# jwscook/DistributedHouseholderQR.jl

Measured on AMD Instinct MI355X. Metric: QR GFLOP/s (F = 2mn^2 - 2/3 n^3), ||A-QR||/||A|| alongside, higher is better.
Workload: dtype f64; 1 GPU; 32768x32768 Float64 dense QR, blocked nb=128 (BASELINE configs[2]); m=32768, n=32768, nb=128, parallelism=single GPU

## Files before the change

### distributedhouseholderqr.jl_amd/_lib.py

```python
from __future__ import annotations

import ctypes
import os
import subprocess

_PKG = os.path.dirname(os.path.abspath(__file__))
SO_PATH = os.path.join(_PKG, "libdhqr.so")
BENCH_SO_PATH = os.path.join(_PKG, "libdhqr_bench.so")
CSRC = os.path.join(_PKG, "csrc")
NB = 128
CS_BLOCK = 256
ZNB = 64

OK, EINVAL, EHIP, ENOMEM, ENODEVICE, ECOMM = 0, -1, -2, -3, -4, -5
COMM_SELF, COMM_RCCL, COMM_LOCAL, COMM_CALLBACK = 0, 1, 2, 3
UNIQUE_ID_BYTES = 128


class DHQRError(RuntimeError):
    def __init__(self, code: int, msg: str):
        super().__init__(f"libdhqr error {code}: {msg}")
        self.code = code


# ... 96 lines not shown
    "dhqr_cs_store_contiguous_f64": (_i32, [_p, _p, _i64, _i64, _i64, _p, _i64, _p]),
    "dhqr_cs_qr_darray_f64": (_i32, [_p, _p, _i64, _i64, _i64, _p]),
    "dhqr_mg_create": (_i32, [_pp, _pi32, _i32]),
    "dhqr_mg_destroy": (_i32, [_p]),
    "dhqr_mg_info": (_i32, [_p, _pi32, _pi32, _pi64, _pi64]),
    "dhqr_mg_get_bcast_tuning": (_i32, [_p, _pi32, _pd, _pd]),
    "dhqr_mg_rccl_nranks": (_i32, [_p, _pi32, _pi32]),
    "dhqr_mg_comm_counters": (_i32, [_p, _i32, _pi64]),
    "dhqr_mg_alloc_f64": (_i32, [_p, _i64, _i64]),
    "dhqr_mg_fill_uniform_f64": (_i32, [_p, _u64]),
    "dhqr_mg_factor_f64": (_i32, [_p]),
    "dhqr_mg_residual_f64": (_i32, [_p, _u64, _pd]),
    "dhqr_mg_upload_f64": (_i32, [_p, _p, _i64, _p]),
    "dhqr_mg_download_f64": (_i32, [_p, _p, _i64, _p]),
    "dhqr_mg_qr_f64": (_i32, [_p, _p, _i64, _i64, _i64, _p]),
    "dhqr_mg_qr_c64": (_i32, [_p, _p, _i64, _i64, _i64, _p]),
    "dhqr_cs_local_cols_c64": (_i64, [_i64, _i32, _i32]),
    "dhqr_cs_factor_c64": (_i32, [_p, _p, _i64, _i64, _i64, _p]),
    "dhqr_cs_qr_darray_c64": (_i32, [_p, _p, _i64, _i64, _i64, _p]),
    "dhqr_comm_timing": (_i32, [_p, _i32, _p]),
    "dhqr_mg_comm_timing": (_i32, [_p, _i32, _i32, _p]),
    "dhqr_cs_ldiv_darray_f64": (_i32, [_p, _p, _i64, _i64, _i64, _p, _p, _p]),
    "dhqr_cs_ldiv_darray_c64": (_i32, [_p, _p, _i64, _i64, _i64, _p, _p, _p]),
    "dhqr_cs_solve_work_c64": (_i64, [_i64, _i32]),
    "dhqr_cs_solve_c64": (_i32, [_p, _p, _i64, _i64, _i64, _p, _p, _p]),
    "dhqr_mg_ldiv_c64": (_i32, [_p, _p, _i64, _i64, _i64, _p, _p, _p]),
    "dhqr_mg_solve_f64": (_i32, [_p, _p, _p]),
    "dhqr_mg_ldiv_f64": (_i32, [_p, _p, _i64, _i64, _i64, _p, _p, _p]),
    "dhqr_mg_set_profiling": (_i32, [_p, _i32]),
    "dhqr_mg_reset_stats": (_i32, [_p]),
    "dhqr_mg_get_stats": (_i32, [_p, _i32, ctypes.POINTER(Stats), _pi64, _pi64, _pi64]),
    "dhqr_rs_row_range": (None, [_i64, _i32, _i32, _pi64, _pi64]),
    "dhqr_rs_fill_uniform_f64": (_i32, [_p, _p, _i64, _i64, _i64, _u64]),
    "dhqr_rs_factor_f64": (_i32, [_p, _p, _i64, _i64, _i64, _p]),
    "dhqr_rs_residual_f64": (_i32, [_p, _p, _i64, _i64, _i64, _p, _u64, _p, _p, _pd]),
    "dhqr_rs_solve_f64": (_i32, [_p, _p, _i64, _i64, _i64, _p, _p, _p]),
    "dhqr_mg_rs_alloc_f64": (_i32, [_p, _i64, _i64]),
    "dhqr_mg_rs_fill_uniform_f64": (_i32, [_p, _u64]),
    "dhqr_mg_rs_factor_f64": (_i32, [_p]),
    "dhqr_mg_rs_residual_f64": (_i32, [_p, _u64, _pd]),
    "dhqr_mg_rs_transfer_f64": (_i32, [_p, _p, _i64, _p, _i32]),
    "dhqr_mg_rs_solve_f64": (_i32, [_p, _p, _p]),
}

BENCH_SIGNATURES = {
    "dhqr_bench_mfma_f64": (_i32, [_p, _pd]),
    "dhqr_bench_issue_f64": (_i32, [_p, _i32, _i32, _pd, _pd]),
    "dhqr_bench_issue2_f64": (_i32, [_p, _i32, _i32, _i32, _pd]),
    "dhqr_bench_stream_f64": (_i32, [_p, _i64, _pd]),
    "dhqr_debug_mfma_probe": (_i32, [_p, _p, _p, _p]),
    "dhqr_bench_gemm_f64": (_i32, [_p, _i32, _i64, _i64, _i32, _pd]),
    "dhqr_bench_mma_probe_f64": (_i32, [_p, _i32, _i32, _pd]),
    "dhqr_bench_lane_probe_f64": (_i32, [_p, _i64, _i32, _i32, _i32, _pd]),
    "dhqr_debug_hold_cus": (_i32, [_p, _i32, _i32, _i32]),
    "dhqr_debug_smq_phases": (_i32, [_p, _pd]),
}

_lib = None


def lib() -> ctypes.CDLL:
    global _lib
    if _lib is None:
        if not os.path.exists(SO_PATH):
            raise ImportError(
                f"{SO_PATH} not found: build it with __graft_entry__.build() "
                "(hipcc --offload-arch=gfx950); this package has no CPU fallback")
        L = ctypes.CDLL(SO_PATH)
        for name, (res, args) in SIGNATURES.items():
            fn = getattr(L, name)
            fn.restype = res
            fn.argtypes = args
        _lib = L
    return _lib


_bench = None


def lib_bench() -> ctypes.CDLL:
    global _bench
    if _bench is None:
        if not os.path.exists(BENCH_SO_PATH):
            raise ImportError(f"{BENCH_SO_PATH} not found: build it with __graft_entry__.build()")
        L = ctypes.CDLL(BENCH_SO_PATH)
        for name, (res, args) in list(SIGNATURES.items()) + list(BENCH_SIGNATURES.items()):
            fn = getattr(L, name)
            fn.restype = res
            fn.argtypes = args
        _bench = L
    return _bench


def check(rc: int) -> None:
    if rc != OK:
        raise DHQRError(rc, lib().dhqr_last_error().decode(errors="replace"))
```

### distributedhouseholderqr.jl_amd/csrc/dhqr_api.hip

```cpp
#include <chrono>
#include <mutex>

#include "dhqr_internal.h"
#include "dhqr_complex.h"
#include "dhqr_gemm.h"
#include "dhqr_pack.h"
#include "dhqr_panel.h"
#include "dhqr_recon.h"
#include "dhqr_solve.h"
#include "dhqr_qtb.h"
#include "dhqr_small.h"
#include "dhqr_batched.h"
#include "dhqr_tsqr.h"

static thread_local char g_err[512] = "";
int32_t set_err(int32_t code, const char *fmt, ...) {
  va_list ap;
  va_start(ap, fmt);
  vsnprintf(g_err, sizeof(g_err), fmt, ap);
  va_end(ap);
  return code;
}
int32_t ensure(dhqr_ctx *c, Buf &b, size_t need) {
  if (need <= b.cap) return DHQR_OK;
  if (b.p) {
    HIPCHECK(hipDeviceSynchronize());
    HIPCHECK(hipFree(b.p));
    b.p = nullptr;
    b.cap = 0;
  }
  need = (need + 1023) & ~(size_t)1023;
  hipError_t e = hipMalloc((void **)&b.p, need * sizeof(double));
  if (e != hipSuccess)
    return set_err(DHQR_ENOMEM, "hipMalloc(%zu bytes) failed: %s", need * sizeof(double),
                   hipGetErrorString(e));
  b.cap = need;
  return DHQR_OK;
}

bool tune_get(const char *key, long long *out) {
  const char *e = getenv("DHQR_TUNE");
  if (!e) return false;
  const size_t kl = strlen(key);
  for (const char *p = e; *p;) {
    const char *q = strchr(p, ',');
    const size_t len = q ? (size_t)(q - p) : strlen(p);
    if (len > kl + 1 && strncmp(p, key, kl) == 0 && p[kl] == '=') {
      *out = atoll(p + kl + 1);
      return true;
    }
    if (!q) break;
    p = q + 1;
  }
  return false;
}

static std::atomic<int> g_live_ctx[64];


int32_t prof_begin(dhqr_ctx *c, int cat) {
  if (!c->profiling) return DHQR_OK;
// ... 527 lines not shown
                                    const PanelBuf &pb, int panel_idx, int part = 0) {
  const size_t NN = (size_t)DHQR_NBV * DHQR_NBV;
  const double *Rref = panel_rbuf(c, panel_idx) + 3 * NN, *altmp = panel_rbuf(c, panel_idx) + 6 * NN;
  if (part == 1) {
    hipLaunchKernelGGL(k_commit_alpha, dim3(1), dim3(DHQR_NBV), 0, stream, altmp, (int)DHQR_NBV, (double *)nullptr, pb.alpha,
                       (const int *)c->dstat, panel_idx);
  } else {
    dim3 grid((unsigned)std::min<int64_t>((rows + 255) / 256, 64), DHQR_NBV);
    hipLaunchKernelGGL(k_commit_panel, grid, dim3(256), 0, stream, P, ldp, rows, (const double *)pb.V, pb.ldv, Rref, altmp, alpha,
                       part == 2 ? (double *)nullptr : pb.alpha, (const int *)c->dstat, panel_idx);
  }
  LAUNCHCHECK();
  return DHQR_OK;
}
static int32_t panel_fast_enqueue(dhqr_ctx *c, double *P, int64_t rows, int64_t ldp, double *alpha, const PanelBuf &pb,
                                  int passes, int panel_idx, hipEvent_t ev_v = nullptr, hipEvent_t ev_t = nullptr) {
  const int64_t ldv = pb.ldv;
  const size_t NN = (size_t)DHQR_NBV * DHQR_NBV;
  CHECK(ensure(c, c->rbuf, 2 * panel_rbuf_elems()));
  if (passes == 2) CHECK(ensure(c, c->vts, (size_t)panel_elems(rows)));
  if (passes == 3) CHECK(ensure(c, c->tsq, TsqrLocal::elems(rows)));
  CHECK(ensure(c, c->sfull, NN));
  if (c->ev_commit[panel_idx & 1]) HIPCHECK(hipStreamWaitEvent(c->stream, c->ev_commit[panel_idx & 1], 0));
  double *R1 = panel_rbuf(c, panel_idx), *negR1inv = R1 + NN, *Rf = R1 + 2 * NN, *Rref = R1 + 3 * NN, *negMinv = R1 + 4 * NN;
  double *G = R1 + 5 * NN, *altmp = R1 + 6 * NN;
  int *bflag = c->dstat + 1;
  CHECK(prof_begin(c, CAT_PANEL));
  const bool was = c->profiling;
  c->profiling = false;
  auto body = [&]() -> int32_t {
    const double *X = P;
    int64_t ldx = ldp;
    if (passes == 3) {
      TsqrLocal t;
      t.place(c->tsq.p, rows);
      CHECK(tsqr_local_up(c, t, P, ldp, Rf, true));
      CHECK(tsqr_local_down(c, t, nullptr));
      hipLaunchKernelGGL(k_tsqr_identity, dim3((unsigned)(NN / 256)), dim3(256), 0, c->stream, R1);
      X = t.Yl;
      ldx = t.ldy;
      launch_recon_top(c, X, ldx, R1, G, Rref, negMinv);
      hipLaunchKernelGGL(k_tsqr_sign_cols, dim3((unsigned)(NN / 256)), dim3(256), 0, c->stream, negMinv, (const double *)Rf);
    } else if (passes == 2) {
      CHECK(gram128(c, P, ldp, rows, G));
      double *Q1 = c->vts.p;
      const int64_t ldq = panel_ldv(rows);
      launch_chol_inv(c, G, nullptr, R1, negR1inv, bflag);
      CHECK(mul128(c, P, ldp, rows, negR1inv, Q1, ldq));
      CHECK(gram128(c, Q1, ldq, rows, G));
      launch_chol_inv(c, G, R1, Rf, nullptr, bflag);
      launch_recon_top(c, P, ldp, Rf, altmp, Rref, negMinv);
    } else {
      CHECK(gram128(c, P, ldp, rows, G));
      hipLaunchKernelGGL((k_panel_top<false>), dim3(1), dim3(1024), 0, c->stream, (const double *)G, (const double *)P, ldp, altmp,
                         Rref, negMinv, bflag);
    }
    if (c->fuse_fix) {
      CHECK(mul128(c, X, ldx, rows, negMinv, pb.V, ldv, passes == 3 ? G : altmp));
    } else {
      CHECK(mul128(c, X, ldx, rows, negMinv, pb.V, ldv));
      hipLaunchKernelGGL(k_recon_fix, dim3(NN / 256), dim3(256), 0, c->stream, pb.V, ldv,
                         (const double *)(passes == 3 ? G : altmp), (const double *)negMinv);
    }
    if (ev_v) HIPCHECK(hipEventRecord(ev_v, c->stream));
    if (passes == 3)
      hipLaunchKernelGGL(k_tsqr_final_r, dim3(NN / 256), dim3(256), 0, c->stream, (const double *)Rf, (const double *)G, Rref,
                         altmp);
    CHECK(gram128(c, pb.V, ldv, rows, c->sfull.p));
    hipLaunchKernelGGL(k_build_t, dim3(1), dim3(1024), 0, c->stream, (const double *)c->sfull.p, (int)DHQR_NBV, pb.T, pb.Tt,
                       c->recon_tol, c->dstat, panel_idx, pb.alpha + DHQR_NBV, c->tt_keep);
    if (ev_t) HIPCHECK(hipEventRecord(ev_t, c->stream));
    else CHECK(panel_commit_enqueue(c, c->stream, P, rows, ldp, alpha, pb, panel_idx));
    LAUNCHCHECK();
    return DHQR_OK;
  };
  const int32_t rc = body();
  c->profiling = was;
  CHECK(rc);
  if (c->profiling)
    for (int64_t j = 0; j + 1 < DHQR_NBV; ++j) c->st.bytes_panel += 16.0 * (double)(rows - j) * (double)(DHQR_NBV - j - 1);
  CHECK(prof_end(c));
  return DHQR_OK;
}
static inline bool panel_fast_eligible(dhqr_ctx *c, int64_t rows, int64_t w) {
  return c->panel_impl == 3 && w == DHQR_NBV && rows >= 2 * DHQR_NBV;
}

static int32_t factor_panel_sync(dhqr_ctx *c, double *P, int64_t rows, int64_t w, int64_t ldp, double *alpha,
                                 const PanelBuf &pb) {
  if (panel_fast_eligible(c, rows, w)) {
    const int last_rung = std::max(c->cholqr_passes, c->tsqr_rung == 1 ? 3 : 2);
    for (int passes = c->cholqr_passes; passes <= last_rung; ++passes) {
      CHECK(status_reset(c));
      CHECK(panel_fast_enqueue(c, P, rows, ldp, alpha, pb, passes, 0));
      int failed = 0;
      CHECK(status_read(c, &failed));
      if (failed == INT_MAX) {
        c->n_fast++;
        if (passes == 3) c->n_tsqr++;
        return DHQR_OK;
      }
    }
    CHECK(status_reset(c));
    c->n_fallback++;
  }
  if (c->panel_impl >= 2 && !(c->partial_unblocked && rows > 256 && rows <= c->partial_unblocked_max_rows))
    return factor_panel_v2(c, P, rows, w, ldp, alpha, pb);
  CHECK(factor_unblocked_cols(c, P, rows, w, ldp, alpha, CAT_PANEL));
  return panel_pack_and_t(c, P, rows, w, ldp, alpha, pb);
}

static int32_t comm_allreduce_sum(dhqr_comm *cm, double *dbuf, int64_t count, hipStream_t stream);

static inline int64_t nn_row_chunks(const dhqr_ctx *c, int64_t row_tiles) {
  if (c->nn_split <= 1 || c->cur_ws != 0) return 1;
  return std::max<int64_t>(1, std::min<int64_t>(c->nn_split, row_tiles / c->nn_chunk_tiles));
}

static int32_t narrow_vtc(dhqr_ctx *c, const double *Vp, int64_t ldv, int64_t rows, const double *C, int64_t ldc,
                          int64_t ncols, bool vec, Buf &part, double *Y) {
  const int64_t ntiles = (ncols + 127) / 128, ld2 = 2 * DHQR_NBV, wstride = ld2 * ncols;
  int64_t nsplit, rps;
  pick_split(rows, 2 * ntiles, 512, 256 / ntiles, &nsplit, &rps, 512, 64);
// ... 419 lines not shown
  HIPCHECK(hipGetDeviceProperties(&prop, device));
  if (strncmp(prop.gcnArchName, "gfx950", 6) != 0)
    return set_err(DHQR_ENODEVICE, "device %d is %s; this library is built for gfx950 only", device,
                   prop.gcnArchName);
  dhqr_ctx *c = new dhqr_ctx();
  c->device = device;
  c->coop = prop.cooperativeLaunch != 0;
  g_live_ctx[device & 63].fetch_add(1);
  memset(&c->st, 0, sizeof(c->st));
  auto init = [&]() -> int32_t {
    HIPCHECK(hipStreamCreateWithFlags(&c->own, hipStreamNonBlocking));
    c->stream = c->own;
    {
      int lo = 0, hi = 0;
      HIPCHECK(hipDeviceGetStreamPriorityRange(&lo, &hi));
      HIPCHECK(hipStreamCreateWithPriority(&c->hi, hipStreamNonBlocking, hi));
      if (const char *e = getenv("DHQR_LANE_SIDE")) c->lane_side = atoi(e) != 0;
      c->hi_priority = hi;
    }
    if (const char *e = getenv("DHQR_LOOKAHEAD")) c->lookahead = atoi(e) != 0;
    {
      int ncu = 0;
      if (hipDeviceGetAttribute(&ncu, hipDeviceAttributeMultiprocessorCount, device) == hipSuccess && ncu > 0) {
        c->rankk_wgs = ncu;
        c->ncu = ncu;
      }
    }
    if (const char *e = getenv("DHQR_SPARE_CUS")) {
      c->spare_cus = std::max(0, std::min(c->ncu - 8, atoi(e)));
      c->spare_cus_set = true;
    }
    if (const char *e = getenv("DHQR_QUAD")) c->quad = atoi(e) != 0;
    if (const char *e = getenv("DHQR_QUAD_MIN_COLS")) c->quad_min_cols = std::max<int64_t>(0, atoll(e));
    { long long v; if (tune_get("rankk_wgs", &v)) c->rankk_wgs = std::max(2, (int)v); }
    if (const char *e = getenv("DHQR_RANKK")) c->rankk = c->rankk_tall = c->rankk_xtall = std::min(5, std::max(1, atoi(e)));
    if (const char *e = getenv("DHQR_RANKK_MAX")) c->rankk_max = std::min(DHQR_RK_KMAX, std::max(1, atoi(e)));
    { long long v; if (tune_get("rankk_max_min_cols", &v)) c->rankk_max_min_cols = std::max(0, (int)v); }
    { long long v; if (tune_get("nn_chunk_tiles", &v)) c->nn_chunk_tiles = std::max(1, (int)v); }
    if (const char *e = getenv("DHQR_NN_SPLIT")) c->nn_split = std::min(16, std::max(1, atoi(e)));
    if (const char *e = getenv("DHQR_RANKK_PIPE")) c->rankk_pipe = std::min(2, std::max(0, atoi(e)));
    { long long v; if (tune_get("tn_min_tiles", &v)) c->tn_model_min_tiles = (int)v; }
    { long long v; if (tune_get("small_flags", &v)) c->small_flags = v != 0; }
    { long long v; if (tune_get("batched_wave", &v)) c->batched_wave = v != 0; }
    { long long v; if (tune_get("short_panel_small", &v)) c->short_panel_small = v != 0; }
    { long long v; if (tune_get("partial_unblocked", &v)) c->partial_unblocked = v != 0; }
    { long long v; if (tune_get("partial_unblocked_max_rows", &v)) c->partial_unblocked_max_rows = v; }
    { long long v; if (tune_get("small_spin_limit", &v)) c->small_spin_limit = (int)v; }
    { long long v; if (tune_get("tn2_rgroups", &v)) c->tn2_rgroups = (int)v; }
    { long long v; if (tune_get("tn2_rg8_rows", &v)) c->tn2_rg8_rows = v; }
    { long long v; if (tune_get("tn2_rg4_rows", &v)) c->tn2_rg4_rows = v; }
    { long long v; if (tune_get("tn2_rg2_rows", &v)) c->tn2_rg2_rows = v; }
    { long long v; if (tune_get("tn_spare", &v)) c->tn_spare = std::max(0, std::min((c->ncu - 8) / 2, (int)v)); }
    { long long v; if (tune_get("tn_spare_cols", &v)) c->tn_spare_cols = v; }
    if (const char *e = getenv("DHQR_PAIR")) c->pair = atoi(e) != 0;
    if (const char *e = getenv("DHQR_PAIR_MIN_N")) c->pair_min_n = atoll(e);
    HIPCHECK(hipHostMalloc((void **)&c->hflag, 4 * sizeof(int), hipHostMallocDefault));
    HIPCHECK(hipMalloc((void **)&c->dstat, 16 * sizeof(int)));
    HIPCHECK(hipMalloc((void **)&c->zflags, DHQR_PIPE_INTS * sizeof(int)));
    HIPCHECK(hipMemsetAsync(c->zflags, 0, DHQR_PIPE_INTS * sizeof(int), c->stream));
    {
      int limit = DHQR_PIPE_SPIN_LIMIT;
      { long long v; if (tune_get("spin_limit", &v)) limit = std::max(1, (int)v); }
      HIPCHECK(hipMemcpyAsync(c->zflags + DHQR_PIPE_LIMIT_OFFSET, &limit, sizeof(int), hipMemcpyHostToDevice, c->stream));
      HIPCHECK(hipStreamSynchronize(c->stream));
    }
    if (const char *e = getenv("DHQR_SMALL")) c->small_route = atoi(e) != 0;
    if (const char *e = getenv("DHQR_ZPIPE")) c->zpipe = atoi(e) != 0;
    if (const char *e = getenv("DHQR_SOLVE_PIPE")) c->solve_pipe = std::max(0, std::min(3, atoi(e)));
    if (const char *e = getenv("DHQR_KEEP_T")) c->keep_t = atoi(e) != 0;
    { long long v; if (tune_get("qtb_vec", &v)) c->qtb_vec = (int)v; }
    { long long v; if (tune_get("gram_strips", &v)) c->gram_strips = v != 0; }
    { long long v; if (tune_get("fuse_fix", &v)) c->fuse_fix = v != 0; }
    { long long v; if (tune_get("commit_off", &v)) c->commit_off = (int)v; }
    hipLaunchKernelGGL(k_set_status, dim3(1), dim3(64), 0, c->stream, c->dstat, INT_MAX);
    LAUNCHCHECK();
    HIPCHECK(hipStreamSynchronize(c->stream));
    return DHQR_OK;
  };
  const int32_t rc_init = init();
  if (rc_init != DHQR_OK) {
    (void)dhqr_destroy(c);
    return rc_init;
  }
  if (const char *e = getenv("DHQR_CHOLQR_PASSES")) c->cholqr_passes = atoi(e) == 2 ? 2 : 1;
  if (const char *e = getenv("DHQR_TSQR")) {
    if (atoi(e) != 0) c->cholqr_passes = 3;
  }
  if (const char *e = getenv("DHQR_TSQR_RUNG")) c->tsqr_rung = atoi(e) != 0 ? 1 : 0;
  if (const char *e = getenv("DHQR_PANEL")) {
    const int v = atoi(e);
    if (v >= 1 && v <= 3) c->panel_impl = v;
  }
  *out = c;
  return DHQR_OK;
}

int32_t dhqr_destroy(dhqr_ctx *c) {
  if (!c) return DHQR_OK;
  g_live_ctx[c->device & 63].fetch_sub(1);
  (void)hipSetDevice(c->device);
  (void)hipStreamSynchronize(c->stream);
  (void)hipDeviceSynchronize();
  cs_state_free(c);
  rs_state_free(c);
  if (c->hio) {
    hio_free(*c->hio);
// ... 2133 lines not shown
```

### distributedhouseholderqr.jl_amd/csrc/dhqr_bench.h

```cpp
#pragma once

__global__ void k_mfma_probe(const double *__restrict__ a, const double *__restrict__ b,
                             double *__restrict__ out) {
  const int lane = threadIdx.x & 63;
  const int i16 = lane & 15, k4 = lane >> 4;
  dhqr_d4 acc = (dhqr_d4){0.0, 0.0, 0.0, 0.0};
  acc = mfma_f64(a[i16 * 4 + k4], b[k4 * 16 + i16], acc);
  for (int g = 0; g < 4; ++g) out[lane * 4 + g] = acc[g];
}

__global__ __launch_bounds__(256) void k_mfma_bench(double *__restrict__ out, int iters) {
  dhqr_d4 acc[16];
  const double a = 1.0 + threadIdx.x * 1e-9, b = 1.0 - threadIdx.x * 1e-9;
#pragma unroll
  for (int x = 0; x < 16; ++x) acc[x] = (dhqr_d4){0.0, 0.0, 0.0, 0.0};
  for (int it = 0; it < iters; ++it) {
#pragma unroll
    for (int x = 0; x < 16; ++x) acc[x] = mfma_f64(a, b, acc[x]);
  }
  double s = 0.0;
#pragma unroll
  for (int x = 0; x < 16; ++x) s += acc[x][0] + acc[x][1] + acc[x][2] + acc[x][3];
  out[(int64_t)blockIdx.x * blockDim.x + threadIdx.x] = s;
}
// ... 463 lines not shown
    HIPCHECK(hipMalloc((void **)&G, (size_t)NB * NB * 8));
    HIPCHECK(hipMalloc((void **)&sink, 1024 * 8));
    HIPCHECK(hipMalloc((void **)&scr, (size_t)(4096 + 4 * NB * NB) * 8));
    for (auto &e : ev) HIPCHECK(hipEventCreate(&e));
    CHECK(dhqr_fill_uniform_f64(c, P, rows, NB, ldp, 5, rows, 0, 128, 1, 0));
    HIPCHECK(hipStreamSynchronize(c->stream));
    HIPCHECK(hipFuncSetAttribute(reinterpret_cast<const void *>(k_lane_standin<8>), hipFuncAttributeMaxDynamicSharedMemorySize, lds_kb * 1024));
    HIPCHECK(hipFuncSetAttribute(reinterpret_cast<const void *>(k_lane_standin<40>), hipFuncAttributeMaxDynamicSharedMemorySize, lds_kb * 1024));
    int64_t rps = (rows + nsplit - 1) / nsplit;
    rps = (rps + G_KT - 1) / G_KT * G_KT;
    const int64_t ns = (rows + rps - 1) / rps;
    double acc[3] = {0.0, 0.0, 0.0};
    for (int r = 0; r <= reps; ++r) {
      HIPCHECK(hipEventRecord(ev[0], st));
      hipLaunchKernelGGL((k_gemm_tn<2, 1, 128>), dim3(1, (unsigned)ns), dim3(256), 0, st, (const double *)P, ldp, (const double *)P, ldp, 1,
                         (int64_t)0, rows, NB, rps, part, NB, NB * NB);
      hipLaunchKernelGGL(k_reduce_splits, dim3((unsigned)(NB * NB / 64)), dim3(256), 0, st, (const double *)part, (int)ns, NB * NB, NB * NB, G);
      HIPCHECK(hipEventRecord(ev[1], st));
      if (real) {
        hipLaunchKernelGGL((k_panel_top<false>), dim3(1), dim3(1024), 0, st, (const double *)G, (const double *)P, ldp, scr, scr + 1024,
                           scr + 1024 + NB * NB, (int *)(scr + 1024 + 2 * NB * NB));
        hipLaunchKernelGGL(k_build_t, dim3(1), dim3(1024), 0, st, (const double *)G, (int)NB, scr + 2048 + 2 * NB * NB, scr + 2048 + 3 * NB * NB,
                           0.0, (int *)nullptr, 0, (double *)nullptr, (double *)nullptr);
      } else if (heavy)
        hipLaunchKernelGGL(k_lane_standin<40>, dim3(1), dim3(1024), (size_t)lds_kb * 1024, st, sink, 128);
      else
        hipLaunchKernelGGL(k_lane_standin<8>, dim3(1), dim3(1024), (size_t)lds_kb * 1024, st, sink, 128);
      HIPCHECK(hipEventRecord(ev[2], st));
      HIPCHECK(hipEventSynchronize(ev[2]));
      float a = 0.f, b = 0.f;
      HIPCHECK(hipEventElapsedTime(&a, ev[0], ev[1]));
      HIPCHECK(hipEventElapsedTime(&b, ev[1], ev[2]));
      if (r > 0) {
        acc[0] += a;
        acc[1] += b;
        acc[2] += a + b;
      }
    }
    LAUNCHCHECK();
    for (int i = 0; i < 3; ++i) out4[i] = acc[i] / reps;
    out4[3] = 0.0;
    return DHQR_OK;
  };
  const int32_t rc = body();
  (void)hipStreamSynchronize(st);
  for (auto &e : ev)
    if (e) (void)hipEventDestroy(e);
  double *ps[] = {P, part, G, sink, scr};
  for (double *p_ : ps)
    if (p_) (void)hipFree(p_);
  return rc;
}

int32_t dhqr_debug_mfma_probe(dhqr_ctx *c, const double *da, const double *db, double *dout) {
  ENTER(c);
  hipLaunchKernelGGL(k_mfma_probe, dim3(1), dim3(64), 0, c->stream, da, db, dout);
  LAUNCHCHECK();
  HIPCHECK(hipStreamSynchronize(c->stream));
  return DHQR_OK;
}

extern "C++" {
__global__ __launch_bounds__(1024) void k_hold_cu(volatile int *release, unsigned long long max_ticks, int *sink) {
  __shared__ int ballast[150 * 1024 / 4];
  if (threadIdx.x == 0) ballast[blockIdx.x & 1023] = 1;
  const unsigned long long t0 = wall_clock64();
  if (threadIdx.x == 0) {
    while (*release == 0 && wall_clock64() - t0 < max_ticks) __builtin_amdgcn_s_sleep(64);
  }
  __syncthreads();
  if (ballast[threadIdx.x] == 12345 && sink) sink[0] = 1;
}
static hipStream_t g_hold_stream = nullptr;
static int *g_hold_flag = nullptr;
}
int32_t dhqr_debug_hold_cus(dhqr_ctx *c, int32_t nwg, int32_t max_ms, int32_t release) {
  ENTER(c);
  if (!g_hold_stream) {
    HIPCHECK(hipStreamCreateWithFlags(&g_hold_stream, hipStreamNonBlocking));
    HIPCHECK(hipHostMalloc((void **)&g_hold_flag, 64, hipHostMallocDefault));
  }
  if (release) {
    *(volatile int *)g_hold_flag = 1;
    HIPCHECK(hipStreamSynchronize(g_hold_stream));
    return DHQR_OK;
  }
  if (nwg < 1 || nwg > 1024 || max_ms < 1 || max_ms > 5000) return set_err(DHQR_EINVAL, "bad arguments");
  *(volatile int *)g_hold_flag = 0;
  hipLaunchKernelGGL(k_hold_cu, dim3((unsigned)nwg), dim3(1024), 0, g_hold_stream, (volatile int *)g_hold_flag,
                     (unsigned long long)max_ms * 100000ull, (int *)nullptr);
  LAUNCHCHECK();
  return DHQR_OK;
}
int32_t dhqr_debug_smq_phases(dhqr_ctx *c, double *out54) {
  ENTER(c);
  unsigned long long h[9][6];
  HIPCHECK(hipStreamSynchronize(c->stream));
  HIPCHECK(hipMemcpyFromSymbol(h, HIP_SYMBOL(g_smq_phase), sizeof(h)));
  for (int w = 0; w < 9; ++w)
    for (int q = 0; q < 6; ++q) out54[w * 6 + q] = (double)h[w][q];
  memset(h, 0, sizeof(h));
  HIPCHECK(hipMemcpyToSymbol(HIP_SYMBOL(g_smq_phase), h, sizeof(h)));
  return DHQR_OK;
}

}
// ... 1 lines not shown
```

### distributedhouseholderqr.jl_amd/csrc/dhqr_dist.h

```cpp
#pragma once

#define CS_NGB 6
#define CS_EVR 8

struct CsState {
  bool init = false;
  hipStream_t comm = nullptr;
  hipEvent_t ev_group[CS_EVR], ev_wide[CS_EVR], ev_head[CS_EVR], ev_lane[CS_EVR];
  hipEvent_t ev_ready[2 * CS_EVR], ev_recv[2 * CS_EVR];
  hipEvent_t ev_v[2 * CS_EVR], ev_y[2 * CS_EVR], ev_x[CS_EVR];
  hipEvent_t ev_t[2 * CS_EVR];
  hipEvent_t ev_start = nullptr, ev_end = nullptr;
  int64_t ticket[2 * CS_EVR];
  Buf gbuf[CS_NGB];
  Buf vt;
};

static int32_t cs_state_init(dhqr_ctx *c) {
  if (!c->cs) c->cs = new CsState();
  CsState &s = *c->cs;
  if (s.init) return DHQR_OK;
  int lo = 0, hi = 0;
  HIPCHECK(hipDeviceGetStreamPriorityRange(&lo, &hi));
  HIPCHECK(hipStreamCreateWithPriority(&s.comm, hipStreamNonBlocking, hi));
// ... 242 lines not shown
      const PanelBuf pbx = idx == 0 ? gb.pa() : gb.pb();
      const int pe = (int)(x % (2 * CS_EVR));
      if (pr.mine(x)) {
        on(sL, 1);
        CHECK(guard(sL));
        const int64_t lc = pr.lcol(x);
        bool was = false;
        if (prev >= 0 && !merged_update) {
          if (second_of_quad) {
            if (sh >= 1) HIPCHECK(hipStreamWaitEvent(sL, (has_head(sh - 1) ? S.ev_head : S.ev_wide)[(sh - 1) % CS_EVR], 0));
          } else if (sh >= 2) {
            const bool in_head = P > 1 && has_head(sh - 2) && h == steps[sh - 2].g0 + steps[sh - 2].ng + 1;
            HIPCHECK(hipStreamWaitEvent(sL, (in_head ? S.ev_head : S.ev_wide)[(sh - 2) % CS_EVR], 0));
          }
          int64_t ncols = w;
          if (gr.np == 2 && idx == 0 && pr.mine(x + 1) && pr.lcol(x + 1) == lc + w) {
            ncols += pr.width(x + 1);
            merged_update = true;
          }
          CHECK(lane_begin(was));
          const int32_t rc = second_of_quad ? apply_group(prev, lc, ncols) : apply_step(sh - 1, lc, ncols);
          CHECK(lane_end(was));
          CHECK(rc);
        }
        if (idx == 1) {
          if (!pr.mine(gr.a)) HIPCHECK(hipStreamWaitEvent(sL, S.ev_recv[(int)(gr.a % (2 * CS_EVR))], 0));
          double *Cb = pr.A + gr.a * NB + lc * lda;
          const int pa_ = (int)(gr.a % (2 * CS_EVR));
          CHECK(lane_begin(was));
          c->epoch = (int)gr.a;
          int32_t rc = DHQR_OK;
          if (side && v_event[0] && (merged_update || prev < 0)) {
            on(sX, 2);
            HIPCHECK(hipStreamWaitEvent(sX, S.ev_v[pa_], 0));
            rc = panel_apply(c, gb.pa(), gb.rows_a, Cb, w, lda, 1, DHQR_NBV, 1);
            HIPCHECK(hipEventRecord(S.ev_y[pa_], sX));
            on(sL, 2);
            HIPCHECK(hipStreamWaitEvent(sL, S.ev_y[pa_], 0));
            if (rc == DHQR_OK) rc = panel_apply(c, gb.pa(), gb.rows_a, Cb, w, lda, 1, DHQR_NBV, 2);
            on(sL, 1);
          } else {
            rc = panel_apply(c, gb.pa(), gb.rows_a, Cb, w, lda, 1);
          }
          CHECK(lane_end(was));
          CHECK(rc);
          hipLaunchKernelGGL(k_zero_rows, dim3(DHQR_NBV), dim3(128), 0, sL, gb.VB, gb.ldv, (int)NB);
        }
        double *Pp = pr.A + x * NB + lc * lda;
        c->epoch = saved_epoch;
        c->tt_keep = (c->tc_base && P == 1) ? c->tc_base + x * (NB * NB) : nullptr;
        bool deferred = false;
        if (panel_fast_eligible(c, rows, w) && !(robust_first && x == kstart)) {
          deferred = sK != nullptr;
          CHECK(panel_fast_enqueue(c, Pp, rows, lda, pr.alpha + x * NB, pbx, c->cholqr_passes, (int)x, side ? S.ev_v[pe] : nullptr,
                                   deferred ? S.ev_t[pe] : nullptr));
          v_event[idx] = side;
          fast_idx.push_back(x);
        } else {
          bool run_it = true;
          if (x != kstart) {
            int f = 0;
            CHECK(status_read(c, &f));
            run_it = (f == INT_MAX);
          }
          if (run_it) CHECK(factor_panel_sync(c, Pp, rows, w, lda, pr.alpha + x * NB, pbx));
          hipLaunchKernelGGL(k_set_statword, dim3(1), dim3(64), 0, sL, (const int *)c->dstat, pbx.alpha + DHQR_NBV);
        }
        c->tt_keep = nullptr;
        auto commit_on = [&](hipStream_t s, int part) -> int32_t {
          CHECK(panel_commit_enqueue(c, s, Pp, rows, lda, pr.alpha + x * NB, pbx, (int)x, part));
          if (part != 1) HIPCHECK(hipEventRecord(c->ev_commit[x & 1], s));
          return DHQR_OK;
        };
        if (deferred && P == 1) {
          HIPCHECK(hipStreamWaitEvent(sK, S.ev_t[pe], 0));
          CHECK(commit_on(sK, 0));
          HIPCHECK(hipEventRecord(S.ev_ready[pe], sK));
        } else if (!deferred) {
          HIPCHECK(hipEventRecord(S.ev_ready[pe], sL));
        }
        if (c->panel_hook && P == 1) CHECK(c->panel_hook(c->panel_hook_arg, x, S.ev_ready[pe]));
        if (cm && P > 1) {
          HIPCHECK(hipStreamWaitEvent(sC, deferred ? S.ev_t[pe] : S.ev_ready[pe], 0));
          if (deferred) CHECK(commit_on(sC, 1));
          CHECK(comm_bcast(cm, gb.region(idx), gb.region_elems(), pr.r, sC, &S.ticket[pe]));
          HIPCHECK(hipEventRecord(S.ev_recv[pe], sC));
          if (deferred) CHECK(commit_on(sC, 2));
        }
      } else {
        CHECK(guard(sC));
        CHECK(comm_bcast(cm, gb.region(idx), gb.region_elems(), pr.owner(x), sC, nullptr));
        hipLaunchKernelGGL(k_adopt_status, dim3(1), dim3(64), 0, sC, (const double *)(pbx.alpha + DHQR_NBV), c->dstat);
        hipLaunchKernelGGL(k_commit_alpha, dim3(1), dim3(DHQR_NBV), 0, sC, (const double *)pbx.alpha, (int)w,
                           pr.alpha + x * NB, (double *)nullptr, (const int *)c->dstat, (int)x);
        HIPCHECK(hipEventRecord(S.ev_recv[pe], sC));
      }
    }
    on(sL, 1);
    for (int idx = 0; idx < gr.np; ++idx)
      if (!pr.mine(gr.a + idx)) HIPCHECK(hipStreamWaitEvent(sL, S.ev_recv[(int)((gr.a + idx) % (2 * CS_EVR))], 0));
    if (gr.np == 2 && gr.last() + 1 < K) {
      bool was = false;
      CHECK(lane_begin(was));
      int32_t rc = DHQR_OK;
      if (side && v_event[1]) {
        const int pb_ = (int)(gr.last() % (2 * CS_EVR));
        on(sX, 2);
        HIPCHECK(hipStreamWaitEvent(sX, S.ev_v[pb_], 0));
// ... 482 lines not shown
```

### distributedhouseholderqr.jl_amd/csrc/dhqr_internal.h

```cpp
#pragma once
#include <hip/hip_runtime.h>

#include <algorithm>
#include <atomic>
#include <climits>
#include <chrono>
#include <cmath>
#include <cstdarg>
#include <cstdio>
#include <cstring>
#include <vector>

#include "../../include/dhqr.h"
#include "dhqr_common.h"

int32_t set_err(int32_t code, const char *fmt, ...);
#define HIPCHECK(expr)                                                                        \
  do {                                                                                        \
    hipError_t e_ = (expr);                                                                   \
    if (e_ != hipSuccess)                                                                     \
      return set_err(DHQR_EHIP, "%s failed: %s (%s:%d)", #expr, hipGetErrorString(e_),        \
                     __FILE__, __LINE__);                                                     \
  } while (0)
#define CHECK(expr)                  \
  do {                               \
    int32_t rc_ = (expr);            \
    if (rc_ != DHQR_OK) return rc_;  \
  } while (0)
#define LAUNCHCHECK() HIPCHECK(hipGetLastError())

enum { CAT_PANEL = 0, CAT_TBUILD, CAT_VTA, CAT_TW, CAT_AVW, CAT_RANK1, CAT_SOLVE, CAT_N };

struct Buf {
  double *p = nullptr;
  size_t cap = 0;
};

struct dhqr_ctx {
  int device = 0;
  hipStream_t own = nullptr, stream = nullptr;
  bool profiling = false;
  hipStream_t hi = nullptr;
  hipStream_t hi2 = nullptr;
  int lane_side = 1;
  int hi_priority = 0;
  int tn_spare = 32;
  int64_t tn_spare_cols = 16384;
  int tn_model_min_tiles = 32;
  int rankk_wgs = 256;
  int rankk = 5;
  int nn_chunk_tiles = 48;
  int nn_split = 4;
  int rankk_pipe = 1;
  int rankk_max_min_cols = 4096;
  int rankk_unfit = 0;
  int rankk_max = 8;
  int rankk_xtall = 5;
  int rankk_tall = 5;
  int ncu = 256;
  int spare_cus = 0;
  bool spare_cus_set = false;
  int quad = 1;
  int64_t quad_min_cols = 10240;
  struct WS { Buf w1, w1r, w2; } ws[3];
  int cur_ws = 0;
  bool lookahead = true;
  Buf vbuf, vt, vts, spart, spart2, sfull, scratch, pbuf;
  Buf zsolve_lo;
  Buf sv_T, sv_S, sv_part, sv_small;
  std::vector<int> sv_units;
  int64_t sv_m = -1, sv_n = -1, sv_rps = 0;
  const int *sv_units_dev = nullptr;
  Buf tc_T, tc_alpha;
  double *tt_keep = nullptr, *tc_base = nullptr;
  const double *tc_A = nullptr;
  int64_t tc_m = 0, tc_n = 0, tc_lda = 0;
  bool tc_valid = false;
  int keep_t = 1;
  int solve_pipe = 1;
  int qtb_vec = -1;
  struct SolveRetry {
    bool valid = false;
    const double *A = nullptr, *alpha = nullptr;
    double *b = nullptr;
    int64_t m = 0, n = 0, lda = 0;
  } retry;
  Buf sv_bkp;
  int64_t n_solve_retry = 0;
  int gram_strips = 1;
  int small_spin_limit = 1 << 20;
  int partial_unblocked = 1;
  int64_t partial_unblocked_max_rows = 4608;
  int short_panel_small = 1;
  int small_flags = 1;
  int tn2_rgroups = 1;
  int64_t tn2_rg8_rows = 20480, tn2_rg4_rows = 10240, tn2_rg2_rows = 5120;
  int fuse_fix = 1;
  int commit_off = -1;
  hipStream_t cstream = nullptr;
  hipEvent_t ev_commit[2] = {nullptr, nullptr};
// ... 49 lines not shown
```

### include/dhqr_bench.h

```cpp
#ifndef DHQR_BENCH_H
#define DHQR_BENCH_H
#include "dhqr.h"
#ifdef __cplusplus
extern "C" {
#endif

int32_t dhqr_bench_mfma_f64(dhqr_ctx *ctx, double *tflops);
int32_t dhqr_bench_stream_f64(dhqr_ctx *ctx, int64_t bytes, double *gbps);
int32_t dhqr_bench_issue_f64(dhqr_ctx *ctx, int32_t kind, int32_t nblocks, double *cycles_per_instr,
                             double *tflops);

int32_t dhqr_debug_mfma_probe(dhqr_ctx *ctx, const double *da, const double *db, double *dout);

int32_t dhqr_bench_issue2_f64(dhqr_ctx *ctx, int32_t mode, int32_t threads, int32_t nblocks, double *out4);

int32_t dhqr_bench_gemm_f64(dhqr_ctx *ctx, int32_t kind, int64_t rows, int64_t ncols, int32_t reps, double *out4);
int32_t dhqr_bench_mma_probe_f64(dhqr_ctx *ctx, int32_t mode, int32_t threads, double *out2);
int32_t dhqr_bench_lane_probe_f64(dhqr_ctx *ctx, int64_t rows, int32_t nsplit, int32_t lds_kb, int32_t reps, double *out4);

int32_t dhqr_debug_hold_cus(dhqr_ctx *ctx, int32_t nwg, int32_t max_ms, int32_t release);
int32_t dhqr_debug_smq_phases(dhqr_ctx *ctx, double *out54);

#ifdef __cplusplus
}
#endif
#endif
```

Before: 60860 GFLOP/s.

## Add compact-LDS slot variants of panel-top and build-T kernels for lookahead panels

Adds new versions of the panel Cholesky/reconstruction kernel and the T-factor builder. They keep the Gram matrix in a packed triangular LDS layout overlaid with the blocked upper-triangular inverse workspace, and do the triangular inverse with f64 MFMA tiles. The goal is a much smaller shared-memory footprint, so these single-workgroup critical-path kernels can share CUs with the concurrent trailing update. They are used for lookahead panels when at least `lane_slot_cols` columns remain, and are on by default. The change also adds a benchmark entry point for timing the kernels in isolation. The risk is that the new numerical path differs slightly, or that the packed-LDS indexing costs more per step than it saves.

```diff
diff --git a/distributedhouseholderqr.jl_amd/_lib.py b/distributedhouseholderqr.jl_amd/_lib.py
--- a/distributedhouseholderqr.jl_amd/_lib.py
+++ b/distributedhouseholderqr.jl_amd/_lib.py
@@ -172,6 +172,7 @@
     "dhqr_bench_gemm_f64": (_i32, [_p, _i32, _i64, _i64, _i32, _pd]),
     "dhqr_bench_mma_probe_f64": (_i32, [_p, _i32, _i32, _pd]),
     "dhqr_bench_lane_probe_f64": (_i32, [_p, _i64, _i32, _i32, _i32, _pd]),
+    "dhqr_bench_lane_kernel_f64": (_i32, [_p, _i32, _i32, _p, _p, _i64, _i64, _i32, ctypes.c_double, _p, _i32, _pd]),
     "dhqr_debug_hold_cus": (_i32, [_p, _i32, _i32, _i32]),
     "dhqr_debug_smq_phases": (_i32, [_p, _pd]),
 }
diff --git a/distributedhouseholderqr.jl_amd/csrc/dhqr_api.hip b/distributedhouseholderqr.jl_amd/csrc/dhqr_api.hip
--- a/distributedhouseholderqr.jl_amd/csrc/dhqr_api.hip
+++ b/distributedhouseholderqr.jl_amd/csrc/dhqr_api.hip
@@ -7,6 +7,7 @@
 #include "dhqr_pack.h"
 #include "dhqr_panel.h"
 #include "dhqr_recon.h"
+#include "dhqr_recon_slot.h"
 #include "dhqr_solve.h"
 #include "dhqr_qtb.h"
 #include "dhqr_small.h"
@@ -640,8 +641,12 @@
       launch_recon_top(c, P, ldp, Rf, altmp, Rref, negMinv);
     } else {
       CHECK(gram128(c, P, ldp, rows, G));
-      hipLaunchKernelGGL((k_panel_top<false>), dim3(1), dim3(1024), 0, c->stream, (const double *)G, (const double *)P, ldp, altmp,
-                         Rref, negMinv, bflag);
+      if (c->lane_slot_now)
+        hipLaunchKernelGGL(k_panel_top_slot, dim3(1), dim3(1024), 0, c->stream, (const double *)G, (const double *)P, ldp, altmp, Rref,
+                           negMinv, bflag);
+      else
+        hipLaunchKernelGGL((k_panel_top<false>), dim3(1), dim3(1024), 0, c->stream, (const double *)G, (const double *)P, ldp, altmp,
+                           Rref, negMinv, bflag);
     }
     if (c->fuse_fix) {
       CHECK(mul128(c, X, ldx, rows, negMinv, pb.V, ldv, passes == 3 ? G : altmp));
@@ -655,8 +660,12 @@
       hipLaunchKernelGGL(k_tsqr_final_r, dim3(NN / 256), dim3(256), 0, c->stream, (const double *)Rf, (const double *)G, Rref,
                          altmp);
     CHECK(gram128(c, pb.V, ldv, rows, c->sfull.p));
-    hipLaunchKernelGGL(k_build_t, dim3(1), dim3(1024), 0, c->stream, (const double *)c->sfull.p, (int)DHQR_NBV, pb.T, pb.Tt,
-                       c->recon_tol, c->dstat, panel_idx, pb.alpha + DHQR_NBV, c->tt_keep);
+    if (passes == 1 && c->lane_slot_now)
+      hipLaunchKernelGGL(k_build_t_slot, dim3(1), dim3(1024), 0, c->stream, (const double *)c->sfull.p, (int)DHQR_NBV, pb.T, pb.Tt,
+                         c->recon_tol, c->dstat, panel_idx, pb.alpha + DHQR_NBV, c->tt_keep);
+    else
+      hipLaunchKernelGGL(k_build_t, dim3(1), dim3(1024), 0, c->stream, (const double *)c->sfull.p, (int)DHQR_NBV, pb.T, pb.Tt,
+                         c->recon_tol, c->dstat, panel_idx, pb.alpha + DHQR_NBV, c->tt_keep);
     if (ev_t) HIPCHECK(hipEventRecord(ev_t, c->stream));
     else CHECK(panel_commit_enqueue(c, c->stream, P, rows, ldp, alpha, pb, panel_idx));
     LAUNCHCHECK();
@@ -1182,6 +1191,8 @@
     { long long v; if (tune_get("tn2_rg2_rows", &v)) c->tn2_rg2_rows = v; }
     { long long v; if (tune_get("tn_spare", &v)) c->tn_spare = std::max(0, std::min((c->ncu - 8) / 2, (int)v)); }
     { long long v; if (tune_get("tn_spare_cols", &v)) c->tn_spare_cols = v; }
+    { long long v; if (tune_get("lane_slot", &v)) c->lane_slot = v < 0 ? -1 : (v > 0 ? 1 : 0); }
+    { long long v; if (tune_get("lane_slot_cols", &v)) c->lane_slot_cols = std::max<long long>(0, v); }
     if (const char *e = getenv("DHQR_PAIR")) c->pair = atoi(e) != 0;
     if (const char *e = getenv("DHQR_PAIR_MIN_N")) c->pair_min_n = atoll(e);
     HIPCHECK(hipHostMalloc((void **)&c->hflag, 4 * sizeof(int), hipHostMallocDefault));
diff --git a/distributedhouseholderqr.jl_amd/csrc/dhqr_bench.h b/distributedhouseholderqr.jl_amd/csrc/dhqr_bench.h
--- a/distributedhouseholderqr.jl_amd/csrc/dhqr_bench.h
+++ b/distributedhouseholderqr.jl_amd/csrc/dhqr_bench.h
@@ -539,6 +539,56 @@
   return rc;
 }
 
+int32_t dhqr_bench_lane_kernel_f64(dhqr_ctx *c, int32_t which, int32_t form, const double *dG, const double *dP, int64_t ldp,
+                                   int64_t rows, int32_t ncols, double tol, double *dout, int32_t reps, double *ms) {
+  ENTER(c);
+  const int64_t NB = DHQR_NBV, NN = NB * NB;
+  if ((which != 0 && which != 1) || (form != 0 && form != 1) || !dout || !ms || reps < 1 || ncols < 1 || ncols > NB || (!dG && !dP) ||
+      (which == 0 && (!dP || ldp < NB)) || (!dG && (rows < NB || ldp < rows)))
+    return set_err(DHQR_EINVAL, "bad arguments");
+  hipEvent_t ev[2] = {nullptr, nullptr};
+  auto body = [&]() -> int32_t {
+    CHECK(ensure(c, c->sfull, (size_t)NN));
+    const double *G = dG;
+    if (!G) {
+      CHECK(gram128(c, dP, ldp, rows, c->sfull.p));
+      G = c->sfull.p;
+    }
+    for (auto &e : ev) HIPCHECK(hipEventCreate(&e));
+    int *words = (int *)(dout + (which == 0 ? NB + 2 * NN : 3 * NN + 1));
+    for (int r = 0; r <= reps; ++r) {
+      if (r == 1) HIPCHECK(hipEventRecord(ev[0], c->stream));
+      if (which == 0) {
+        HIPCHECK(hipMemsetAsync(words, 0, 2 * sizeof(int), c->stream));
+        if (form == 0)
+          hipLaunchKernelGGL((k_panel_top<false>), dim3(1), dim3(1024), 0, c->stream, G, dP, ldp, dout, dout + NB, dout + NB + NN, words);
+        else
+          hipLaunchKernelGGL(k_panel_top_slot, dim3(1), dim3(1024), 0, c->stream, G, dP, ldp, dout, dout + NB, dout + NB + NN, words);
+      } else {
+        hipLaunchKernelGGL(k_set_status, dim3(1), dim3(64), 0, c->stream, words, INT_MAX);
+        if (form == 0)
+          hipLaunchKernelGGL(k_build_t, dim3(1), dim3(1024), 0, c->stream, G, (int)ncols, dout, dout + NN, tol, words, 5, dout + 3 * NN,
+                             dout + 2 * NN);
+        else
+          hipLaunchKernelGGL(k_build_t_slot, dim3(1), dim3(1024), 0, c->stream, G, (int)ncols, dout, dout + NN, tol, words, 5, dout + 3 * NN,
+                             dout + 2 * NN);
+      }
+    }
+    HIPCHECK(hipEventRecord(ev[1], c->stream));
+    LAUNCHCHECK();
+    HIPCHECK(hipEventSynchronize(ev[1]));
+    float t = 0.f;
+    HIPCHECK(hipEventElapsedTime(&t, ev[0], ev[1]));
+    *ms = (double)t / reps;
+    return DHQR_OK;
+  };
+  const int32_t rc = body();
+  (void)hipStreamSynchronize(c->stream);
+  for (auto &e : ev)
+    if (e) (void)hipEventDestroy(e);
+  return rc;
+}
+
 int32_t dhqr_debug_mfma_probe(dhqr_ctx *c, const double *da, const double *db, double *dout) {
   ENTER(c);
   hipLaunchKernelGGL(k_mfma_probe, dim3(1), dim3(64), 0, c->stream, da, db, dout);
diff --git a/distributedhouseholderqr.jl_amd/csrc/dhqr_dist.h b/distributedhouseholderqr.jl_amd/csrc/dhqr_dist.h
--- a/distributedhouseholderqr.jl_amd/csrc/dhqr_dist.h
+++ b/distributedhouseholderqr.jl_amd/csrc/dhqr_dist.h
@@ -318,8 +318,11 @@
         bool deferred = false;
         if (panel_fast_eligible(c, rows, w) && !(robust_first && x == kstart)) {
           deferred = sK != nullptr;
-          CHECK(panel_fast_enqueue(c, Pp, rows, lda, pr.alpha + x * NB, pbx, c->cholqr_passes, (int)x, side ? S.ev_v[pe] : nullptr,
-                                   deferred ? S.ev_t[pe] : nullptr));
+          c->lane_slot_now = c->lane_slot != 0 && sh >= 1 && pr.ncl - lc >= c->lane_slot_cols;
+          const int32_t rc_fast = panel_fast_enqueue(c, Pp, rows, lda, pr.alpha + x * NB, pbx, c->cholqr_passes, (int)x,
+                                                     side ? S.ev_v[pe] : nullptr, deferred ? S.ev_t[pe] : nullptr);
+          c->lane_slot_now = false;
+          CHECK(rc_fast);
           v_event[idx] = side;
           fast_idx.push_back(x);
         } else {
diff --git a/distributedhouseholderqr.jl_amd/csrc/dhqr_internal.h b/distributedhouseholderqr.jl_amd/csrc/dhqr_internal.h
--- a/distributedhouseholderqr.jl_amd/csrc/dhqr_internal.h
+++ b/distributedhouseholderqr.jl_amd/csrc/dhqr_internal.h
@@ -46,6 +46,9 @@
   int hi_priority = 0;
   int tn_spare = 32;
   int64_t tn_spare_cols = 16384;
+  int lane_slot = -1;
+  int64_t lane_slot_cols = 16384;
+  bool lane_slot_now = false;
   int tn_model_min_tiles = 32;
   int rankk_wgs = 256;
   int rankk = 5;
diff --git a/distributedhouseholderqr.jl_amd/csrc/dhqr_recon_slot.h b/distributedhouseholderqr.jl_amd/csrc/dhqr_recon_slot.h
--- /dev/null
+++ b/distributedhouseholderqr.jl_amd/csrc/dhqr_recon_slot.h
@@ -0,0 +1,275 @@
+#pragma once
+#include "dhqr_recon.h"
+
+#if defined(__AMDGCN__)
+#define RCS_OPAQUE(v) asm volatile("" : "+v"(v))
+#else
+#define RCS_OPAQUE(v) do { } while (0)
+#endif
+
+struct rcs_lds {
+  double W[4 * 32 * RC5_LDD];
+  double X[65][66];
+  double dinv[RC_N];
+};
+__device__ __forceinline__ double rcs_xh(const rcs_lds &L, int h, int i, int j) {
+  return (i <= j) ? (h == 0 ? L.X[i][j] : L.X[j + 1][i]) : 0.0;
+}
+__device__ __forceinline__ void rcs_xh_put(rcs_lds &L, int h, int i, int j, double v) {
+  if (i <= j) {
+    if (h == 0) L.X[i][j] = v;
+    else L.X[j + 1][i] = v;
+  }
+}
+#define RCS_UD(d, i, l) L.W[((d) * 32 + (i)) * RC5_LDD + (l)]
+#define RCS_T1A(r, c) L.W[2 * 32 * RC5_LDD + (r) * RC5_LDD + (c)]
+#define RCS_T1B(r, c) L.W[(r) * RC5_LDH + (c)]
+
+__device__ __forceinline__ void rcs_upper_inverse_blocked(const double *__restrict__ Mg, int ncols, bool unit, rcs_lds &L,
+                                                          double (&x12)[4], const double *rs = nullptr) {
+  int t = threadIdx.x;
+  RCS_OPAQUE(t);
+#pragma unroll
+  for (int r = 0; r < 4; ++r) {
+    const int e = t + 1024 * r, d = e >> 10, i = e & 31, l = (e >> 5) & 31;
+    RCS_UD(d, i, l) = rc5_in(Mg, 32 * d + i, 32 * d + l, ncols, rs);
+  }
+  if (t < RC_N) L.dinv[t] = unit ? 1.0 : 1.0 / (rs ? rs[RC_N + t] : Mg[t + t * RC_N]);
+  __syncthreads();
+  if (t < RC_N) {
+    const int d = t >> 5, hb = (t >> 4) & 1, k = t & 15, q = 16 * hb;
+    double x[16];
+#pragma unroll
+    for (int i = 15; i >= 0; --i) {
+      double s = 0.0;
+#pragma unroll
+      for (int l = i + 1; l < 16; ++l) s = fma(RCS_UD(d, q + i, q + l), x[l], s);
+      x[i] = (i == k) ? L.dinv[32 * d + q + k] : ((i < k) ? -s * L.dinv[32 * d + q + i] : 0.0);
+    }
+    const int h = d >> 1, o = (d & 1) * 32 + q;
+#pragma unroll
+    for (int i = 0; i < 16; ++i) rcs_xh_put(L, h, o + i, o + k, x[i]);
+  }
+  __syncthreads();
+  if (t < 256) {
+    const int d = t >> 6, ln = t & 63, pi = ln & 15, pk = ln >> 4, h = d >> 1, o = (d & 1) * 32;
+    dhqr_d4 tb = (dhqr_d4){0.0, 0.0, 0.0, 0.0};
+#pragma unroll
+    for (int ks = 0; ks < 4; ++ks)
+      tb = __builtin_amdgcn_mfma_f64_16x16x4f64(RCS_UD(d, pi, 16 + 4 * ks + pk), rcs_xh(L, h, o + 16 + 4 * ks + pk, o + 16 + pi), tb, 0, 0, 0);
+    dhqr_d4 xb = (dhqr_d4){0.0, 0.0, 0.0, 0.0};
+#pragma unroll
+    for (int ks = 0; ks < 4; ++ks)
+      xb = __builtin_amdgcn_mfma_f64_16x16x4f64(rcs_xh(L, h, o + pi, o + 4 * ks + pk), tb[ks], xb, 0, 0, 0);
+#pragma unroll
+    for (int g = 0; g < 4; ++g) rcs_xh_put(L, h, o + pk + 4 * g, o + 16 + pi, -xb[g]);
+  }
+  __syncthreads();
+  double b3[4];
+#pragma unroll
+  for (int r = 0; r < 4; ++r) {
+    const int e = t + 1024 * r;
+    b3[r] = rc5_in(Mg, e & 63, 64 + (e >> 6), ncols, rs);
+  }
+  {
+    const int i = t & 31, l = t >> 5;
+    RCS_UD(0, i, l) = rc5_in(Mg, i, 32 + l, ncols, rs);
+    RCS_UD(1, i, l) = rc5_in(Mg, 64 + i, 96 + l, ncols, rs);
+  }
+  __syncthreads();
+  const int lane = t & 63, w = t >> 6, fi = lane & 15, fk = lane >> 4;
+  {
+    const int h = w >> 2, ti = (w >> 1) & 1, tj = w & 1;
+    if (w < 8) {
+      dhqr_d4 acc = (dhqr_d4){0.0, 0.0, 0.0, 0.0};
+#pragma unroll
+      for (int ks = 0; ks < 8; ++ks)
+        acc = __builtin_amdgcn_mfma_f64_16x16x4f64(RCS_UD(h, 16 * ti + fi, 4 * ks + fk), rcs_xh(L, h, 32 + 4 * ks + fk, 32 + 16 * tj + fi),
+                                                  acc, 0, 0, 0);
+#pragma unroll
+      for (int g = 0; g < 4; ++g) RCS_T1A(32 * h + 16 * ti + fk + 4 * g, 16 * tj + fi) = acc[g];
+    }
+    __syncthreads();
+    dhqr_d4 acc = (dhqr_d4){0.0, 0.0, 0.0, 0.0};
+    if (w < 8) {
+#pragma unroll
+      for (int ks = 0; ks < 8; ++ks)
+        acc = __builtin_amdgcn_mfma_f64_16x16x4f64(rcs_xh(L, h, 16 * ti + fi, 4 * ks + fk), RCS_T1A(32 * h + 4 * ks + fk, 16 * tj + fi), acc, 0,
+                                                  0, 0);
+    }
+    if (w < 8) {
+#pragma unroll
+      for (int g = 0; g < 4; ++g) rcs_xh_put(L, h, 16 * ti + fk + 4 * g, 32 + 16 * tj + fi, -acc[g]);
+    }
+    __syncthreads();
+#pragma unroll
+    for (int r = 0; r < 4; ++r) {
+      const int e = t + 1024 * r;
+      L.W[(e & 63) * RC5_LDH + (e >> 6)] = b3[r];
+    }
+  }
+  __syncthreads();
+  {
+    const int ti = w & 3, tj = w >> 2;
+    dhqr_d4 acc = (dhqr_d4){0.0, 0.0, 0.0, 0.0};
+#pragma unroll
+    for (int ks = 0; ks < 16; ++ks)
+      acc = __builtin_amdgcn_mfma_f64_16x16x4f64(L.W[(16 * ti + fi) * RC5_LDH + 4 * ks + fk], rcs_xh(L, 1, 4 * ks + fk, 16 * tj + fi), acc, 0, 0,
+                                                0);
+    __syncthreads();
+#pragma unroll
+    for (int g = 0; g < 4; ++g) RCS_T1B(16 * ti + fk + 4 * g, 16 * tj + fi) = acc[g];
+    __syncthreads();
+    acc = (dhqr_d4){0.0, 0.0, 0.0, 0.0};
+#pragma unroll
+    for (int ks = 0; ks < 16; ++ks)
+      acc = __builtin_amdgcn_mfma_f64_16x16x4f64(rcs_xh(L, 0, 16 * ti + fi, 4 * ks + fk), RCS_T1B(4 * ks + fk, 16 * tj + fi), acc, 0, 0, 0);
+#pragma unroll
+    for (int g = 0; g < 4; ++g) x12[g] = -acc[g];
+  }
+}
+template <typename F>
+__device__ __forceinline__ void rcs_emit(const rcs_lds &L, const double (&x12)[4], F &&put) {
+  int t = threadIdx.x;
+  RCS_OPAQUE(t);
+#pragma unroll
+  for (int r = 0; r < 4; ++r) {
+    const int e = t + 1024 * r, i = e & 63, j = e >> 6;
+    put(i, j, rcs_xh(L, 0, i, j));
+    put(64 + i, 64 + j, rcs_xh(L, 1, i, j));
+    put(16 * ((t >> 6) & 3) + ((t & 63) >> 4) + 4 * r, 64 + 16 * (t >> 8) + (t & 15), x12[r]);
+    put(64 + i, j, 0.0);
+  }
+}
+
+__global__ __launch_bounds__(1024, 8) void k_build_t_slot(const double *__restrict__ S, int ncols, double *__restrict__ Tout,
+                                                           double *__restrict__ Ttout, double tol, int *__restrict__ stat,
+                                                           int panel_idx, double *__restrict__ statword,
+                                                           double *__restrict__ Tt2) {
+  __shared__ rcs_lds L;
+  __shared__ int bad[RC_N];
+  if (stat != nullptr) {
+    const int j = threadIdx.x;
+    if (j < RC_N) bad[j] = (fabs(S[j + j * RC_N] - 2.0) <= tol) ? 0 : 1;
+    __syncthreads();
+    if (j == 0) {
+      int any = stat[1];
+      for (int q = 0; q < RC_N; ++q) any |= bad[q];
+      if (any && stat[0] > panel_idx) stat[0] = panel_idx;
+      stat[1] = 0;
+      if (statword) *statword = (double)stat[0];
+    }
+  }
+  double x12[4];
+  rcs_upper_inverse_blocked(S, ncols, true, L, x12);
+  rcs_emit(L, x12, [&](int i, int k, double v) {
+    Tout[i + k * RC_N] = v;
+    Ttout[k + i * RC_N] = v;
+    if (Tt2) Tt2[k + i * RC_N] = v;
+  });
+}
+
+#define RCS_G_ELEMS (6 * 1024 + 2 * 33 * 32)
+static_assert(sizeof(rcs_lds) >= RCS_G_ELEMS * sizeof(double), "the Gram matrix is overlaid with the inverse's arrays");
+__device__ __forceinline__ int rcs_g_at(int x, int y, int ti, int tk) {
+  if (x == y) return 6 * 1024 + (x >> 1) * (33 * 32) + ((x & 1) ? (tk + 1) * 32 + ti : ti * 32 + tk);
+  return (x * (7 - x) / 2 + (y - x - 1)) * 1024 + ti * 32 + tk;
+}
+
+__global__ __launch_bounds__(1024, 8) void k_panel_top_slot(const double *__restrict__ G, const double *__restrict__ P,
+                                                             int64_t ldp, double *__restrict__ alpha,
+                                                             double *__restrict__ Rref, double *__restrict__ negMinv,
+                                                             int *__restrict__ flag) {
+  __shared__ double rbuf[2 * RC_N], wrow[2 * RC_N], vcol[2 * RC_N], qu[2 * RC_N];
+  __shared__ rcs_lds L;
+  double *gl = &L.W[0];
+  const int t = threadIdx.x;
+  double a[4][4];
+  {
+    int tt = t;
+    RCS_OPAQUE(tt);
+    const int ti = tt >> 5, tk = tt & 31;
+#pragma unroll
+    for (int x = 0; x < 4; ++x)
+#pragma unroll
+      for (int y = 0; y < 4; ++y) {
+        if (y > x || (y == x && ti <= tk)) gl[rcs_g_at(x, y, ti, tk)] = G[(ti + 32 * x) + (tk + 32 * y) * RC_N];
+        a[x][y] = P[(ti + 32 * x) + (int64_t)(tk + 32 * y) * ldp];
+      }
+  }
+#pragma unroll
+  for (int ja = 0; ja < 4; ++ja)
+    for (int jm = 0; jm < 32; ++jm) {
+      const int j = ja * 32 + jm;
+      int tt = t;
+      RCS_OPAQUE(tt);
+      const int ti = tt >> 5, tk = tt & 31, lane = tt & 63;
+      const int src = (lane & 32) + jm;
+      const double gd = (ti == tk) ? gl[rcs_g_at(ja, ja, ti, tk)] : 0.0;
+      double d = __shfl(gd, src, 64);
+      const double ajj = __shfl(a[ja][ja], src, 64);
+      double *rb = rbuf + (j & 1) * RC_N, *wr = wrow + (j & 1) * RC_N, *vc = vcol + (j & 1) * RC_N;
+      if (ti == jm) {
+        if (!(d > 0.0)) {
+          if (tk == 0) flag[0] = 1;
+          d = 1.0;
+        }
+        double r, rinv;
+        dhqr_sqrt_rsqrt(d, r, rinv);
+        const double al = r * dhqr_alphafactor(ajj);
+        const double u = dhqr_rcp(ajj - al);
+        if (tk == 0) {
+          qu[j] = r * (r + fabs(ajj));
+          qu[RC_N + j] = u;
+        }
+        const double sg = (al == 0.0) ? 0.0 : (al < 0.0 ? -1.0 : 1.0);
+#pragma unroll
+        for (int y = 0; y < 4; ++y) {
+          const int k = tk + 32 * y;
+          const double gv = (k > j) ? gl[rcs_g_at(ja, y, ti, tk)] : 0.0;
+          const double x = (k == j) ? r : gv * rinv;
+          rb[k] = (k > j) ? x : 0.0;
+          const double rr = sg * x;
+          const double dl = (k > j) ? (a[ja][y] - rr) : 0.0;
+          wr[k] = dl * u;
+          negMinv[j + k * RC_N] = dl;
+          Rref[j + k * RC_N] = (k > j) ? rr : 0.0;
+        }
+        if (tk == 0) alpha[j] = al;
+      }
+      if (tk == jm) {
+#pragma unroll
+        for (int x = 0; x < 4; ++x) {
+          const int i = ti + 32 * x;
+          vc[i] = (i > j) ? a[x][ja] : 0.0;
+        }
+      }
+      __syncthreads();
+#pragma unroll
+      for (int x = 0; x < 4; ++x) {
+        if (x < ja) continue;
+        const double ri = rb[ti + 32 * x], vi = vc[ti + 32 * x];
+#pragma unroll
+        for (int y = 0; y < 4; ++y) {
+          if (y < ja) continue;
+          const double rk = rb[tk + 32 * y];
+          if (y > x || (y == x && ti <= tk)) {
+            const int at = rcs_g_at(x, y, ti, tk);
+            gl[at] = fma(-ri, rk, gl[at]);
+          }
+          a[x][y] = fma(-vi, wr[tk + 32 * y], a[x][y]);
+        }
+      }
+    }
+  __syncthreads();
+  if (t < RC_N) {
+    const double sq = sqrt(qu[t]);
+    qu[t] = sq * qu[RC_N + t];
+    qu[RC_N + t] = sq;
+  }
+  __syncthreads();
+  double x12[4];
+  rcs_upper_inverse_blocked(negMinv, RC_N, false, L, x12, qu);
+  __syncthreads();
+  rcs_emit(L, x12, [&](int i, int k, double v) { negMinv[i + k * RC_N] = -v; });
+}
diff --git a/include/dhqr_bench.h b/include/dhqr_bench.h
--- a/include/dhqr_bench.h
+++ b/include/dhqr_bench.h
@@ -18,6 +18,9 @@
 int32_t dhqr_bench_mma_probe_f64(dhqr_ctx *ctx, int32_t mode, int32_t threads, double *out2);
 int32_t dhqr_bench_lane_probe_f64(dhqr_ctx *ctx, int64_t rows, int32_t nsplit, int32_t lds_kb, int32_t reps, double *out4);
 
+int32_t dhqr_bench_lane_kernel_f64(dhqr_ctx *ctx, int32_t which, int32_t form, const double *dG, const double *dP, int64_t ldp,
+                                   int64_t rows, int32_t ncols, double tol, double *dout, int32_t reps, double *ms);
+
 int32_t dhqr_debug_hold_cus(dhqr_ctx *ctx, int32_t nwg, int32_t max_ms, int32_t release);
 int32_t dhqr_debug_smq_phases(dhqr_ctx *ctx, double *out54);
 
```

Measured after the change: 61220 GFLOP/s (median of 6 runs). No clear change (+0.6%).
